# bacpop/Pansim

Hardware: AMD Instinct MI355X
Metric: generations/sec (higher is better)
Workload: dtype u8

## Files before the change

### pansim_amd/csrc/core_kernels.h

```cpp
#pragma once

#include "ps_common.h"

#include <type_traits>

#define PS_SWEEP_MAX_GENS 2
struct core_sweep_args {
    uint8_t *state;
    uint8_t *out;
    const uint32_t *idx;
    const uint32_t *idx_next[PS_SWEEP_MAX_GENS - 1];
    const uint32_t *idxT;
    uint32_t N, pitch, cpr, rows;
    uint32_t site_offset;
    uint32_t gen, k0, k1;
    ps_core_plan plan;
    uint32_t *overflow_flag;
    unsigned long long *stamps;
    uint32_t *work_ctr;
    uint32_t launch_parity;
    uint32_t nt;
    uint32_t qcap;
    uint32_t qcap_limit;
    uint32_t *wide_flags;
// ... 123 lines not shown
                    d[j] = w;
                }
            } else {
                const uint4 v = *(const uint4 *)(grow + 16u * c);
                d[0] = v.x; d[1] = v.y; d[2] = v.z; d[3] = v.w;
            }
            uint32_t hm = 0;
            if (events) {
                const ps_u4 A = ps_philox_l1a(site >> 1, c, a.gen, a.k0, a.k1), B = ps_philox_l1b(site >> 2, c, a.gen, a.k0, a.k1);
                uint32_t cm = ps_cand_word(A, site, pl.cshift);
                while (cm) {
                    const uint32_t k = ps_bit_cell(__builtin_ctz(cm));
                    cm &= cm - 1u;
                    const uint32_t i = c * 16u + k;
                    if (i >= a.N) continue;
                    uint32_t l2y;
                    const ps_cell cell = ps_cell_events<WT>(a, A, B, site, i, a.gen, a.k0, a.k1, pl, l2y);
                    if (DO_MUT && cell.mut) ps_set_byte(d, k, cell.mut);
                    if (DO_HR && cell.hr) hm |= 1u << k;
                }
            }
            if (DO_HR) {
                *(uint4 *)(rowS + 16u * c) = make_uint4(d[0], d[1], d[2], d[3]);
                hrm[c] = (uint16_t)hm;
            } else {
                *(uint4 *)(grow + 16u * c) = make_uint4(d[0], d[1], d[2], d[3]);
            }
        }
        if (DO_HR) {
            __syncthreads();
            for (uint32_t c = lane; c < a.cpr; c += lpr) {
                const uint4 v = *(const uint4 *)(rowS + 16u * c);
                uint32_t d[4] = { v.x, v.y, v.z, v.w };
                uint32_t hm = hrm[c];
                while (hm) {
                    const uint32_t k = __builtin_ctz(hm);
                    hm &= hm - 1u;
                    const uint32_t i = c * 16u + k;
                    const ps_u4 l2 = ps_philox(site, i, a.gen, PS_STREAM_CORE_L2, a.k0, a.k1);
                    uint32_t donor = ps_mulhi(l2.y, a.N - 1u);
                    donor += (donor >= i) ? 1u : 0u;
                    ps_set_byte(d, k, (uint32_t)rowS[donor]);
                }
                *(uint4 *)(grow + 16u * c) = make_uint4(d[0], d[1], d[2], d[3]);
            }
            if (!DO_GATHER) __syncthreads();
        }
    }
}

#define PS_BATCH_ROWS 4u

__device__ __forceinline__ void ps_wave_sync()
{
    __builtin_amdgcn_fence(__ATOMIC_RELEASE, "wavefront");
    __builtin_amdgcn_wave_barrier();
    __builtin_amdgcn_fence(__ATOMIC_ACQUIRE, "wavefront");
}

__device__ __forceinline__ uint32_t ps_lane_prefix(uint64_t bal)
{
    return __builtin_amdgcn_mbcnt_hi((uint32_t)(bal >> 32), __builtin_amdgcn_mbcnt_lo((uint32_t)bal, 0u));
}

__device__ __forceinline__ uint32_t ps_wave_scan_incl(uint32_t x)
{
    x += (uint32_t)__builtin_amdgcn_update_dpp(0, (int)x, 0x111, 0xF, 0xF, false);
    x += (uint32_t)__builtin_amdgcn_update_dpp(0, (int)x, 0x112, 0xF, 0xF, false);
    x += (uint32_t)__builtin_amdgcn_update_dpp(0, (int)x, 0x114, 0xF, 0xF, false);
    x += (uint32_t)__builtin_amdgcn_update_dpp(0, (int)x, 0x118, 0xF, 0xF, false);
    x += (uint32_t)__builtin_amdgcn_update_dpp(0, (int)x, 0x142, 0xA, 0xF, false);
    x += (uint32_t)__builtin_amdgcn_update_dpp(0, (int)x, 0x143, 0xC, 0xF, false);
    return x;
}

struct ps_class_words { uint32_t dec, res; };
__device__ __forceinline__ ps_class_words ps_classes(uint32_t p0, uint32_t p1, uint32_t p2, uint32_t p3, uint32_t p4, uint32_t p5,
                                                     uint32_t k, uint32_t nE, uint32_t vm)
{
    const uint32_t c1 = __builtin_amdgcn_bitop3_b32(p1, p2, p3, 0x01) & vm;
    uint32_t lt;
    switch (nE) {
    case 1: lt = __builtin_amdgcn_bitop3_b32(p0, p5, p4, 0x01); break;
    case 2: lt = __builtin_amdgcn_bitop3_b32(p0, p5, p4, 0x03); break;
    case 3: lt = __builtin_amdgcn_bitop3_b32(p0, p5, p4, 0x07); break;
    case 4: lt = __builtin_amdgcn_bitop3_b32(p0, p5, p4, 0x0F); break;
    case 5: lt = __builtin_amdgcn_bitop3_b32(p0, p5, p4, 0x1F); break;
    case 6: lt = __builtin_amdgcn_bitop3_b32(p0, p5, p4, 0x3F); break;
    case 7: lt = __builtin_amdgcn_bitop3_b32(p0, p5, p4, 0x7F); break;
    default: lt = 0xFFFFFFFFu; break;
    }
    ps_class_words o;
    o.dec = k ? c1 & __builtin_amdgcn_bitop3_b32(p0, p5, p4, 0x07) : 0u;
    o.res = c1 & lt & ~o.dec;
    return o;
}

struct ps_apply_words { uint32_t y0, y1, ya, yb, yc; };
PS_HD uint32_t ps_bfi(uint32_t m, uint32_t a, uint32_t b)
{
#if defined(__HIP_DEVICE_COMPILE__) && __has_builtin(__builtin_amdgcn_bitop3_b32)
    return __builtin_amdgcn_bitop3_b32(m, a, b, 0xCA);
#else
    return (a & m) | (b & ~m);
#endif
}
__device__ __forceinline__ ps_apply_words ps_apply_prepare(uint32_t dec, uint32_t p4, uint32_t p5)
{
    const uint32_t r1 = p5 >> 1, r2 = p4 >> 2, l1 = p5 << 1, l2 = dec << 2;
    ps_apply_words o;
    o.y0 = ps_bfi(0x01010101u, p4, ps_bfi(0x02020202u, l1, l2));
    o.y1 = ps_bfi(0x02020202u, p4, ps_bfi(0x04040404u, l1, l2));
    o.ya = ps_bfi(0x09090909u, r2, ps_bfi(0x12121212u, r1, dec));
    o.yb = ps_bfi(0x12121212u, r2, ps_bfi(0x24242424u, r1, dec));
    o.yc = ps_bfi(0x24242424u, r2, ps_bfi(0x48484848u, r1, dec));
    return o;
}
template <uint32_t SLOT>
__device__ __forceinline__ uint32_t ps_apply_dword(const ps_apply_words &y, uint32_t d)
{
    constexpr uint32_t sh = SLOT == 0u ? 0u : SLOT == 1u ? 1u : SLOT == 2u ? 0u : SLOT == 3u ? 1u : SLOT == 4u ? 2u : SLOT == 5u ? 3u : SLOT == 6u ? 4u : 5u;
    const uint32_t src = SLOT == 0u ? y.y0 : SLOT == 1u ? y.y1 : (SLOT == 2u || SLOT == 5u) ? y.ya : (SLOT == 3u || SLOT == 6u) ? y.yb : y.yc;
    const uint32_t f = (src >> sh) & 0x07070707u;
    const uint32_t allele = __builtin_amdgcn_perm(0x00080402u, 0u, f);
    const uint32_t mask = __builtin_amdgcn_perm(0x00FFFFFFu, 0u, f);
    return ps_bfi(mask, allele, d);
}
template <uint32_t H>
__device__ __forceinline__ void ps_apply_row(const ps_apply_words &y, uint4 &d)
{
    d.x = ps_apply_dword<4u * H + 0u>(y, d.x);
    d.y = ps_apply_dword<4u * H + 1u>(y, d.y);
    d.z = ps_apply_dword<4u * H + 2u>(y, d.z);
    d.w = ps_apply_dword<4u * H + 3u>(y, d.w);
}

__device__ __forceinline__ uint32_t ps_push_scan(uint32_t w0, uint32_t w1, uint16_t *q, uint32_t lane, uint32_t qcap)
{
    const uint32_t c0 = (uint32_t)__popc(w0), c = c0 + (uint32_t)__popc(w1);
    const uint32_t incl = ps_wave_scan_incl(c);
    const uint32_t qn = __builtin_amdgcn_readlane(incl, 63);
    if (qn <= qcap) {
        uint16_t *qp = q + (incl - c) - 1, *qp1 = qp + c0;
        const uint32_t tag = lane << 6;
        for (uint32_t m = w0; m; m &= m - 1u) *++qp = (uint16_t)(tag | (uint32_t)__builtin_ctz(m));
        for (uint32_t m = w1; m; m &= m - 1u) *++qp1 = (uint16_t)(tag | 32u | (uint32_t)__builtin_ctz(m));
    }
    return qn;
}
__device__ __forceinline__ uint32_t ps_entry_cell(uint32_t ent)
{
    const uint32_t cell = ((ent & 3u) << 2) | ((ent >> 3) & 3u), row = ((ent >> 2) & 1u) | ((ent >> 4) & 2u);
    return (row << 10) | ((ent >> 2) & 0x3F0u) | cell;
}

__device__ __forceinline__ uint32_t ps_pack4(uint32_t b0, uint32_t b1, uint32_t b2, uint32_t b3)
{
    return __builtin_amdgcn_perm(b1, b0, 0x0c0c0400u) | __builtin_amdgcn_perm(b3, b2, 0x04000c0cu);
}

#ifdef PS_STAMP
#define PS_T(k) do { unsigned long long t_; asm volatile("s_waitcnt lgkmcnt(0)\n\ts_memtime %0\n\ts_waitcnt lgkmcnt(0)" : "=s"(t_) :: "memory"); st_acc[k] += t_ - st_last; st_last = t_; } while (0)
#else
#define PS_T(k) do { } while (0)
#endif
#ifndef PS_WAVE_LB
#define PS_WAVE_LB 6
#endif
#ifndef PS_WAVE_PREFETCH
#define PS_WAVE_PREFETCH 0
#endif
__host__ __device__ constexpr uint32_t ps_queue_bytes(uint32_t qcap) { return (qcap * 2u + 15u) & ~15u; }
__host__ __device__ constexpr uint32_t ps_wave_lds(uint32_t qcap) { return PS_BATCH_ROWS * 1024u + ps_queue_bytes(qcap); }

template <bool DO_GATHER, bool DO_MUT, bool DO_HR, bool NT = false, bool WT = false, uint32_t T = 1>
__global__ void __launch_bounds__(256, T > 1 ? 4 : PS_WAVE_LB) core_sweep_wave_kernel(core_sweep_args a)
{
    static_assert(T >= 1 && T <= PS_SWEEP_MAX_GENS, "generations per pass");
    static_assert(T == 1 || (DO_GATHER && (DO_MUT || DO_HR)), "several generations per pass: the gather + events form only");
#ifdef PS_STAMP
    unsigned long long st_acc[8] = { 0, 0, 0, 0, 0, 0, 0, 0 };
    unsigned long long st_last;
    asm volatile("s_memtime %0\n\ts_waitcnt lgkmcnt(0)" : "=s"(st_last) :: "memory");
#endif
#ifdef PS_GROUP_TIMES
    const unsigned long long gt_start = __builtin_amdgcn_s_memrealtime();
#endif
    constexpr uint32_t PS_ROWS = PS_BATCH_ROWS;
    extern __shared__ __attribute__((aligned(16))) uint8_t lds[];
    const uint32_t wave = threadIdx.x >> 6, lane = threadIdx.x & 63u;
    uint8_t *rowbuf = lds + wave * ps_wave_lds(a.qcap);
    uint16_t *q = (uint16_t *)(rowbuf + PS_ROWS * 1024u);
    const ps_core_plan pl = a.plan;
    const uint32_t nE = 3u * pl.k + pl.R;
    constexpr bool events = DO_MUT || DO_HR;
    const bool has_chunk = lane < a.cpr;
    const uint32_t i0 = lane * 16u;
    const uint32_t ld_off = has_chunk ? i0 : 0u;
    const uint32_t nvalid = (i0 >= a.N) ? 0u : min(16u, a.N - i0);
    const uint32_t vm = ps_valid_word(nvalid);

    uint32_t pidx[T][16];
    if (DO_GATHER) {
#pragma unroll
        for (uint32_t t = 0; t < T; t++) {
            const uint32_t *ix = t ? a.idx_next[t ? t - 1u : 0u] : a.idx;
#pragma unroll
            for (uint32_t k = 0; k < 16; k++) pidx[t][k] = (k < nvalid) ? ix[i0 + k] : min(a.N, a.pitch - 1u);
        }
    }

    constexpr uint32_t PS_CHUNK = 3u;
    const uint32_t grp = blockIdx.x & 7u;
    const uint32_t off = a.site_offset & 3u, g0 = a.site_offset >> 2;
    const uint32_t batches = (a.rows + off + PS_ROWS - 1u) / PS_ROWS;
    const uint32_t b_lo = (uint32_t)((uint64_t)batches * grp / 8u), b_hi = (uint32_t)((uint64_t)batches * (grp + 1u) / 8u);
    uint32_t *ctr = a.work_ctr + (a.launch_parity * 8u + grp) * 32u;
    if (blockIdx.x < 8u && threadIdx.x == 0) a.work_ctr[((a.launch_parity ^ 1u) * 8u + blockIdx.x) * 32u] = 0u;
    uint32_t next_chunk = 0;
    if (lane == 0) next_chunk = __hip_atomic_fetch_add(ctr, 1u, __ATOMIC_RELAXED, __HIP_MEMORY_SCOPE_AGENT);
#if PS_WAVE_PREFETCH
    uint4 vn[PS_ROWS];
    uint32_t pf_batch = 0xFFFFFFFFu;
#pragma unroll
    for (uint32_t rr = 0; rr < PS_ROWS; rr++) vn[rr] = make_uint4(0, 0, 0, 0);
#endif
    for (;;) {
        const uint32_t chunk = __builtin_amdgcn_readfirstlane(next_chunk);
        if (b_lo + chunk * PS_CHUNK >= b_hi) break;
        if (lane == 0) next_chunk = __hip_atomic_fetch_add(ctr, 1u, __ATOMIC_RELAXED, __HIP_MEMORY_SCOPE_AGENT);
    for (uint32_t cb = 0; cb < PS_CHUNK; cb++) {
        const uint32_t batch = b_lo + chunk * PS_CHUNK + cb;
        if (batch >= b_hi) break;
        const int lr0 = (int)(batch * PS_ROWS) - (int)off;
        const uint32_t sg = g0 + batch;
        auto lrow = [&](uint32_t rr) -> uint32_t { return (uint32_t)min(max(lr0 + (int)rr, 0), (int)a.rows - 1); };
        uint4 v[PS_ROWS];
#if PS_WAVE_PREFETCH
        if (pf_batch == batch) {
#pragma unroll
            for (uint32_t rr = 0; rr < PS_ROWS; rr++) v[rr] = vn[rr];
        } else
#endif
#pragma unroll
        for (uint32_t rr = 0; rr < PS_ROWS; rr++)
            v[rr] = ps_load_row16(a.state + (size_t)lrow(rr) * a.pitch + ld_off, NT);
        if (DO_GATHER) {
#pragma unroll
            for (uint32_t rr = 0; rr < PS_ROWS; rr++) *(uint4 *)(rowbuf + rr * 1024u + i0) = v[rr];
            ps_wave_sync();
        }
        PS_T(0);

#pragma unroll
        for (uint32_t t = 0; t < T; t++) {
        const uint32_t gen = a.gen + t;
        uint32_t wl[2] = { 0u, 0u };
        ps_apply_words y[2] = {};
        if (events) {
            const ps_u4 A0 = ps_philox_l1a(2u * sg, lane, gen, a.k0, a.k1);
            const ps_u4 A1 = ps_philox_l1a(2u * sg + 1u, lane, gen, a.k0, a.k1);
            const ps_u4 B = ps_philox_l1b(sg, lane, gen, a.k0, a.k1);
            const ps_class_words c0 = ps_classes(A0.x, A0.y, A0.z, A0.w, B.x, B.z, pl.k, nE, vm);
            const ps_class_words c1 = ps_classes(A1.x, A1.y, A1.z, A1.w, B.y, B.w, pl.k, nE, vm);
            wl[0] = c0.res;
            wl[1] = c1.res;
            if (DO_MUT) {
                y[0] = ps_apply_prepare(c0.dec, B.x & c0.dec, B.z & c0.dec);
                y[1] = ps_apply_prepare(c1.dec, B.y & c1.dec, B.w & c1.dec);
            }
        }
        PS_T(2);
#pragma unroll
        for (uint32_t rr = 0; rr < PS_ROWS; rr++) {
            uint8_t *row = rowbuf + rr * 1024u;
            uint4 d = v[rr];
            if (DO_GATHER) {
                uint32_t w[4];
#pragma unroll
                for (int j = 0; j < 4; j++)
                    w[j] = ps_pack4(row[pidx[t][4 * j]], row[pidx[t][4 * j + 1]], row[pidx[t][4 * j + 2]], row[pidx[t][4 * j + 3]]);
                d = make_uint4(w[0], w[1], w[2], w[3]);
            }
            if (events && DO_MUT) {
                if (rr & 1u) ps_apply_row<1u>(y[rr >> 1], d);
                else ps_apply_row<0u>(y[rr >> 1], d);
            }
            if (DO_GATHER) ps_wave_sync();
            if (DO_GATHER || events) *(uint4 *)(row + i0) = d;
            __builtin_amdgcn_sched_barrier(0);
        }
        PS_T(1);
        const uint32_t qcap = a.qcap_limit ? min(a.qcap, a.qcap_limit) : a.qcap;
        uint32_t qn = 0;
        if (events) qn = ps_push_scan(wl[0], wl[1], q, lane, qcap);
        PS_T(3);
        ps_wave_sync();
#if PS_WAVE_PREFETCH
        if (t + 1u == T) {
            uint32_t nb = batch + 1u;
            if (cb + 1u >= PS_CHUNK || nb >= b_hi) nb = b_lo + (uint32_t)__builtin_amdgcn_readfirstlane(next_chunk) * PS_CHUNK;
            pf_batch = nb < b_hi ? nb : 0xFFFFFFFFu;
            if (nb < b_hi) {
                const int nlr0 = (int)(nb * PS_ROWS) - (int)off;
#pragma unroll
                for (uint32_t rr = 0; rr < PS_ROWS; rr++)
                    vn[rr] = ps_load_row16(a.state + (size_t)(uint32_t)min(max(nlr0 + (int)rr, 0), (int)a.rows - 1) * a.pitch + ld_off, NT);
            }
        }
#endif
        const bool redo = events && (qn > qcap || (DO_HR && 2u * qn > qcap));
        if (redo) {
#pragma unroll 1
            for (uint32_t rr = 0; rr < PS_ROWS; rr++) {
                uint8_t *row = rowbuf + rr * 1024u;
                const uint32_t site = 4u * sg + rr;
                const ps_u4 Ar = ps_philox_l1a(site >> 1, lane, gen, a.k0, a.k1);
                const ps_u4 Br = ps_philox_l1b(sg, lane, gen, a.k0, a.k1);
                uint32_t cmr = ps_cand_word(Ar, site, pl.cshift) & vm;
                uint32_t hm = 0;
                while (cmr) {
                    const uint32_t k = ps_bit_cell(__builtin_ctz(cmr)), cellidx = i0 + k;
                    cmr &= cmr - 1u;
                    uint32_t l2y = 0;
                    const ps_cell cell = ps_cell_events<WT>(a, Ar, Br, site, cellidx, gen, a.k0, a.k1, pl, l2y);
                    if (DO_MUT && cell.mut) row[cellidx] = (uint8_t)cell.mut;
                    if (DO_HR && cell.hr) hm |= 1u << k;
                }
                if (DO_HR) {
                    ps_wave_sync();
                    uint32_t dv[4] = { 0u, 0u, 0u, 0u };
                    for (uint32_t tmp = hm; tmp;) {
                        const uint32_t k = __builtin_ctz(tmp), cellidx = i0 + k;
                        tmp &= tmp - 1u;
                        const ps_u4 l2 = ps_philox(site, cellidx, gen, PS_STREAM_CORE_L2, a.k0, a.k1);
                        uint32_t donor = ps_mulhi(l2.y, a.N - 1u);
                        donor += (donor >= cellidx) ? 1u : 0u;
                        ps_set_byte(dv, k, (uint32_t)row[donor]);
                    }
                    ps_wave_sync();
                    for (uint32_t tmp = hm; tmp;) {
                        const uint32_t k = __builtin_ctz(tmp);
                        tmp &= tmp - 1u;
                        row[i0 + k] = (uint8_t)((dv[k >> 2] >> (8u * (k & 3u))) & 0xFFu);
                    }
                }
            }
            ps_wave_sync();
        } else if (events) {
            uint16_t *qh = q + qcap - 1u;
            for (uint32_t base = 0; base < qn; base += 64u) {
                const uint32_t e = base + lane;
                if (e < qn) {
                    const uint32_t ent = ps_entry_cell(q[e]);
                    const uint32_t cellidx = ent & 1023u, rr = ent >> 10;
                    const ps_u4 l2 = ps_philox(4u * sg + rr, cellidx, gen, PS_STREAM_CORE_L2, a.k0, a.k1);
                    const ps_cell cell = ps_classify_site<WT>(l2.x, pl, a, 4u * sg + rr);
                    if (DO_MUT && cell.mut) rowbuf[ent] = (uint8_t)cell.mut;
                    if (DO_HR) {
                        uint32_t out = 0;
                        if (cell.hr) {
                            uint32_t donor = ps_mulhi(l2.y, a.N - 1u);
                            donor += (donor >= cellidx) ? 1u : 0u;
                            out = donor | 0x8000u;
                        }
                        *(qh - e) = (uint16_t)out;
                    }
                }
            }
            if (DO_HR) {
                ps_wave_sync();
                for (uint32_t base = 0; base < qn; base += 64u) {
                    const uint32_t e = base + lane;
                    if (e < qn) {
                        const uint32_t h = *(qh - e);
                        if (h >> 15) *(qh - e) = (uint16_t)((uint32_t)rowbuf[(ps_entry_cell(q[e]) & 3072u) | (h & 1023u)] | 0x8000u);
                    }
                }
                ps_wave_sync();
                for (uint32_t base = 0; base < qn; base += 64u) {
                    const uint32_t e = base + lane;
                    if (e < qn) {
                        const uint32_t h = *(qh - e);
                        if (h >> 15) rowbuf[ps_entry_cell(q[e])] = (uint8_t)(h & 0xFFu);
                    }
                }
            }
            ps_wave_sync();
        }
        }
        PS_T(5);

        if (has_chunk) {
#pragma unroll
            for (uint32_t rr = 0; rr < PS_ROWS; rr++) {
                const int lr = lr0 + (int)rr;
                if (lr >= 0 && lr < (int)a.rows) {
                    const uint4 o = (DO_GATHER || events) ? *(const uint4 *)(rowbuf + rr * 1024u + i0) : v[rr];
                    ps_store_row16(a.out + (size_t)lr * a.pitch + i0, o, NT);
                }
            }
        }
        ps_wave_sync();
        PS_T(6);
    }
    }
#ifdef PS_STAMP
    if (lane == 0)
        for (int k = 0; k < 8; k++) atomicAdd((unsigned long long *)a.stamps + k, st_acc[k]);
#endif
#ifdef PS_GROUP_TIMES
    if (lane == 0) {
        atomicMax((unsigned long long *)a.stamps + 8 + grp, (unsigned long long)__builtin_amdgcn_s_memrealtime());
        atomicMax((unsigned long long *)a.stamps + 16 + grp, gt_start);
        if (blockIdx.x < 8 && wave == 0) ((unsigned long long *)a.stamps)[24 + grp] = gt_start;
    }
#endif
}

#ifndef PS_WCAP
#define PS_WCAP 1216u
#endif
#ifndef PS_WBPC
#define PS_WBPC 6
#endif
#ifndef PS_WLB
#define PS_WLB 6
#endif
#ifndef PS_WINDOW_NT_LOADS
#define PS_WINDOW_NT_LOADS 0
#endif
#define PS_WSTRIDE (PS_WCAP + 16u)
#define PS_WHR 64u
__host__ __device__ constexpr uint32_t ps_window_lds(uint32_t qcap) { return PS_BATCH_ROWS * PS_WSTRIDE + ps_queue_bytes(qcap) + PS_WHR * 6u; }

template <bool WT>
__device__ __forceinline__ uint32_t ps_donor_value(const core_sweep_args &a, const ps_core_plan &pl, const uint8_t *old_row,
                                                   uint32_t site, uint32_t donor, bool do_mut)
{
    uint32_t val = old_row[a.idx[donor]];
    if (do_mut) {
        const ps_u4 A = ps_philox_l1a(site >> 1, donor >> 4, a.gen, a.k0, a.k1);
// ... 1631 lines not shown
```

### pansim_amd/csrc/pansim_capi.hip

```cpp
#include "../../include/pansim_hip.h"

#include <hip/hip_runtime.h>

#include <algorithm>
#include <charconv>
#include <chrono>
#include <condition_variable>
#include <mutex>
#include <cmath>
#include <cstdarg>
#include <cstdio>
#include <cstdlib>
#include <cstring>
#include <string>
#include <thread>
#include <type_traits>
#include <vector>

#include "acc_kernels.h"
#include "core_kernels.h"
#include "ps_common.h"

static thread_local std::string g_err;

// ... 3054 lines not shown
    int32_t *h_num_genes = nullptr, *m_num_genes = nullptr;
    double *h_logw = nullptr, *m_logw = nullptr, *h_avg = nullptr;
    double *d_avg = nullptr;
    bool avg_prefetched = false;
    uint64_t avg_epoch = 0;
    hipEvent_t ev_avg = nullptr;
    std::vector<double> h_w;
    hipEvent_t ev_bin = nullptr;
    double *d_log1p = nullptr;
    uint64_t step_count = 0;
    uint64_t gens_done = 0;
    bool need_logw = false;
    bool device_draw = false;
    double *h_cum = nullptr, *d_cum = nullptr;
    uint32_t *d_idx_tsum = nullptr;
    uint32_t *d_idx_cnt = nullptr;
    int last_slot = 0;
    uint32_t *d_anc = nullptr;
    uint32_t anc_capacity = 0;
    uint64_t anc_written = 0;
    uint32_t *h_cnt = nullptr;
    uint64_t h_cnt_cap = 0;
    hipEvent_t ev_dist[4] = {};
    double dist_core_ms = 0.0, dist_acc_ms = 0.0;
    uint64_t host_calls = 0;
    double host_wait_ms = 0.0, host_weights_ms = 0.0, host_draw_ms = 0.0;
    int (*weights_hook)(void *ctx, ps_sim *s, uint32_t gen, double *w) = nullptr;
    void *weights_ctx = nullptr;
    int emu_shards = 0;
    void *emu_buf = nullptr;
    uint64_t emu_cap = 0;
    uint32_t emu_clock_khz = 0;
    double emu_link_gbps = 153.0, emu_latency_us = 20.0, emu_modelled_us = 0.0;
    uint64_t exchange_calls = 0, exchange_bytes = 0;
    bool timing = false;
    std::vector<std::pair<hipEvent_t, hipEvent_t>> tev;
    std::vector<hipEvent_t> ev_pool;
};

extern "C" void ps_sim_destroy(ps_sim *s)
{
    if (!s) return;
    if (s->core) (void)hipSetDevice(s->core->device);
    if (s->core) (void)hipStreamSynchronize(s->core->stream);
    if (s->acc) (void)hipStreamSynchronize(s->acc->stream);
    for (int k = 0; k < PS_RING; k++) {
        if (s->d_idx[k]) (void)hipFree(s->d_idx[k]);
        if (s->h_idx[k]) (void)hipHostFree(s->h_idx[k]);
        if (s->h_draw[k]) (void)hipHostFree(s->h_draw[k]);
        if (s->ev_idx[k]) (void)hipEventDestroy(s->ev_idx[k]);
        if (s->ev_core[k]) (void)hipEventDestroy(s->ev_core[k]);
        if (k == 0 && s->ev_hgt) (void)hipEventDestroy(s->ev_hgt);
        if (k == 0 && s->ev_avg) (void)hipEventDestroy(s->ev_avg);
        if (k == 0 && s->ev_bin) (void)hipEventDestroy(s->ev_bin);
        for (int j = 0; j < 2; j++) if (s->ev_gap[k][j]) (void)hipEventDestroy(s->ev_gap[k][j]);
    }
    if (s->h_num_genes) (void)hipHostFree(s->h_num_genes);
    if (s->h_logw) (void)hipHostFree(s->h_logw);
    if (s->h_avg) (void)hipHostFree(s->h_avg);
    if (s->h_cum) (void)hipHostFree(s->h_cum);
    if (s->d_cum) (void)hipFree(s->d_cum);
    if (s->d_idx_cnt) (void)hipFree(s->d_idx_cnt);
    if (s->d_idx_tsum) (void)hipFree(s->d_idx_tsum);
    if (s->d_anc) (void)hipFree(s->d_anc);
    if (s->h_cnt) (void)hipHostFree(s->h_cnt);
    for (auto e : s->ev_dist) if (e) (void)hipEventDestroy(e);
    if (s->d_avg) (void)hipFree(s->d_avg);
    if (s->emu_buf) (void)hipFree(s->emu_buf);
    if (s->d_log1p) (void)hipFree(s->d_log1p);
    for (auto &pr : s->tev) { (void)hipEventDestroy(pr.first); (void)hipEventDestroy(pr.second); }
    for (auto e : s->ev_pool) (void)hipEventDestroy(e);
    ps_population_destroy(s->core);
    ps_population_destroy(s->acc);
    delete s;
}

static int sim_refresh_rows(void *ctx);
static uint32_t sim_sweep_generations(ps_sim *s);

static int sim_create_impl(const ps_sim_params *p, ps_sim *s)
{
    char msg[1024];
    if (ps_sim_validate(p, msg, sizeof msg) != PS_OK) return ps_fail(PS_ERR_INVALID, "%s", msg);
    if (p->shard_count < 1 || p->shard_rank < 0 || p->shard_rank >= p->shard_count)
        return ps_fail(PS_ERR_INVALID, "bad shard %d of %d", p->shard_rank, p->shard_count);
    if (p->pop_size < 2) return ps_fail(PS_ERR_INVALID, "pop_size must be >= 2 (main.rs:421 / population.rs:584 panic)");
    s->prm = *p;
    PSCHK(ps_sim_derive(p, &s->der));
    const ps_derived &d = s->der;
    const uint64_t N = p->pop_size, L = p->core_size, G = d.pan_size;
    s->sel.assign(std::max<uint64_t>(G, 1), 0.0);
    if (p->reference_seed_stream)
        PSCHK(ps_reference_selection_coefficients(p->seed, G, p->prop_positive, p->pos_lambda, p->neg_lambda, s->sel.data()));
    else
        PSCHK(ps_selection_coefficients(p->seed, G, p->prop_positive, p->pos_lambda, p->neg_lambda, s->sel.data()));
    for (uint64_t g = 0; g < G; g++)
        if (std::log(1.0 + s->sel[g]) != 0.0) s->need_logw = true;
    const uint64_t sb = L * (uint64_t)p->shard_rank / (uint64_t)p->shard_count;
    const uint64_t se = L * ((uint64_t)p->shard_rank + 1) / (uint64_t)p->shard_count;
    ps_config cc{};
    cc.pop_size = N; cc.ncols = se - sb; cc.global_cols = L; cc.col_offset = sb;
    cc.core_genes = p->core_genes; cc.seed = p->seed; cc.core = 1; cc.device = p->device;
    {
        std::vector<uint8_t> v(std::max<uint64_t>(cc.ncols, 1));
        PSCHK(ps_init_vector(p->seed, 1, sb, cc.ncols, 0.0, v.data()));
        PSCHK(ps_population_create(&cc, v.data(), &s->core));
    }
    ps_config ca{};
    ca.pop_size = N; ca.ncols = G; ca.global_cols = G; ca.col_offset = 0;
    ca.core_genes = p->core_genes; ca.seed = p->seed; ca.core = 0; ca.device = s->core->device;
    {
        std::vector<uint8_t> v(std::max<uint64_t>(G, 1));
        PSCHK(ps_init_vector(p->seed, 0, 0, G, d.avg_gene_freq_adj, v.data()));
        PSCHK(ps_population_create(&ca, v.data(), &s->acc));
    }
    s->core->rows_refresh = s->acc->rows_refresh = sim_refresh_rows;
    s->core->rows_ctx = s->acc->rows_ctx = s;
    {
        const uint64_t b0 = 0, e0 = L;
        const double lm = d.n_core_mutations;
        const double lr = (p->HR_rate > 0.0) ? d.n_recombinations_core : 0.0;
        PSCHK(ps_set_rates(s->core, 1, &lm, &lr, &b0, &e0));
        double lrec[2] = { 0, 0 };
        for (int c = 0; c < d.n_comp; c++) lrec[c] = (p->HGT_rate > 0.0) ? d.n_recombinations_pan[c] : 0.0;
        PSCHK(ps_set_rates(s->acc, d.n_comp, d.n_pan_mutations, lrec, d.comp_begin, d.comp_end));
    }
    s->r1.resize(p->max_distances);
    s->r2.resize(p->max_distances);
    PSCHK(ps_sample_pairs(p->seed, N, p->max_distances, s->r1.data(), s->r2.data()));
    PSCHK(use_device(s->core));
    for (int k = 0; k < PS_RING; k++) {
        HIPCHK(hipMalloc(&s->d_idx[k], N * sizeof(uint32_t)));
        HIPCHK(hipHostMalloc(&s->h_idx[k], N * sizeof(uint32_t), hipHostMallocMapped));
        HIPCHK(hipHostGetDevicePointer((void **)&s->m_idx[k], s->h_idx[k], 0));
        HIPCHK(hipHostMalloc(&s->h_draw[k], N * sizeof(uint32_t), hipHostMallocMapped));
        HIPCHK(hipHostGetDevicePointer((void **)&s->m_draw[k], s->h_draw[k], 0));
        HIPCHK(hipEventCreateWithFlags(&s->ev_idx[k], hipEventDisableTiming));
        HIPCHK(hipEventCreateWithFlags(&s->ev_core[k], hipEventDisableTiming));
    }
    if (p->max_distances > 0) {
        PSCHK(upload_pairs(s->core, p->max_distances, s->r1.data(), s->r2.data(), true));
        PSCHK(upload_pairs(s->acc, p->max_distances, s->r1.data(), s->r2.data(), true));
    }
    if (!wave_sweep_eligible(s->core, true, p->HR_rate > 0.0)) {
        core_block_geom g{};
        uint32_t lds = 0, nw = 0;
        if (block_sweep_geometry(s->core, true, true, p->HR_rate > 0.0, &g, &lds, &nw))
            s->acc->hgt_list_in_global = lds + 16384u > s->core->lds_limit;
    }
    {
        const double bytes = 2.0 * (double)N * (double)s->core->cfg.ncols;
        double ept;
        if (sim_sweep_generations(s) >= 2u) {
            const double per_gen_ms = bytes / 3.7e12 * 1e3 / 2.0;
            ept = std::min((0.95 * per_gen_ms - 0.25) / 0.4e-3, 192.0);
        } else {
            const double sweep_ms = bytes / 4.2e12 * 1e3;
            ept = std::min((sweep_ms - 0.3) / 1.0e-3 * 0.5, 112.0);
        }
        s->acc->hgt_events_per_thread = ept >= 16.0 ? (uint32_t)ept : 0u;
        if (const char *e = getenv("PANSIM_HGT_EVENTS_PER_THREAD")) s->acc->hgt_events_per_thread = (uint32_t)atoi(e);
    }
    HIPCHK(hipEventCreateWithFlags(&s->ev_hgt, hipEventDisableTiming));
    {
        const uint32_t parts = hgt_partitions(s->acc);
        s->heavy_hgt = (double)N * s->der.n_recombinations_pan_total >= 7.5e6 && parts >= 1 && parts <= 1024;
    }
    if (const char *e = getenv("PANSIM_HEAVY_HGT")) s->heavy_hgt = atoi(e) != 0;
    if (!getenv("PANSIM_SWEEP_BLOCKS_PER_CU")) {
        uint64_t max_comp = 0;
        for (int c = 0; c < d.n_comp; c++) max_comp = std::max<uint64_t>(max_comp, d.comp_end[c] - d.comp_begin[c]);
        const uint64_t list_lds = 2 * max_comp;
        if (list_lds > 36 * 1024) s->acc->hgt_list_in_global = true;
        const uint32_t light = 4u;
        s->core->sweep_blocks_per_cu = list_lds <= 16 * 1024 ? light : std::min(light, 6u);
    }
    HIPCHK(hipHostMalloc(&s->h_num_genes, N * sizeof(int32_t), hipHostMallocMapped));
    HIPCHK(hipHostMalloc(&s->h_logw, N * sizeof(double), hipHostMallocMapped));
    HIPCHK(hipHostGetDevicePointer((void **)&s->m_num_genes, s->h_num_genes, 0));
    HIPCHK(hipHostGetDevicePointer((void **)&s->m_logw, s->h_logw, 0));
    HIPCHK(hipHostMalloc(&s->h_avg, N * sizeof(double)));
    s->device_draw = N >= 4096;
    if (const char *e = getenv("PANSIM_DEVICE_DRAW")) s->device_draw = atoi(e) != 0;
    HIPCHK(hipHostMalloc(&s->h_cum, N * sizeof(double)));
    HIPCHK(hipMalloc(&s->d_cum, N * sizeof(double)));
    HIPCHK(hipMalloc(&s->d_idx_tsum, ((N + 1023) / 1024 + 1) * sizeof(uint32_t)));
    HIPCHK(hipMalloc(&s->d_idx_cnt, N * sizeof(uint32_t)));
    HIPCHK(hipMemset(s->d_idx_cnt, 0, N * sizeof(uint32_t)));
    HIPCHK(hipMalloc(&s->d_avg, N * sizeof(double)));
    if (G) {
        std::vector<double> l1p(G);
        for (uint64_t g = 0; g < G; g++) l1p[g] = std::log(1.0 + s->sel[g] * 1.0);
        HIPCHK(hipMalloc(&s->d_log1p, G * sizeof(double)));
        HIPCHK(hipMemcpy(s->d_log1p, l1p.data(), G * sizeof(double), hipMemcpyHostToDevice));
    }
    if (G && !s->need_logw && !(getenv("PANSIM_FUSE_COUNTS") && atoi(getenv("PANSIM_FUSE_COUNTS")) == 0)) {
        s->acc->fuse_counts_out = s->m_num_genes;
        s->acc->fuse_logw_out = s->m_logw;
    }
    return PS_OK;
}

extern "C" int ps_sim_create(const ps_sim_params *p, ps_sim **out)
{
    if (!p || !out) return ps_fail(PS_ERR_INVALID, "null argument");
    *out = nullptr;
    ps_sim *s = new ps_sim();
    const int rc = sim_create_impl(p, s);
    if (rc != PS_OK) {
        const std::string keep = g_err;
        ps_sim_destroy(s);
        g_err = keep;
        return rc;
    }
    *out = s;
    return PS_OK;
}

static int sim_average_distance(ps_sim *s)
{
    ps_population *acc = s->acc;
    const uint64_t N = s->prm.pop_size;
    hipStream_t sa = acc->stream;
    const bool sharded = acc->exchange && acc->donor_cnt != 0 && acc->d.G > 0 && N >= 2;
    if (!sharded) return average_distance_device(acc, s->d_avg, sa);
    HIPCHK(hipMemsetAsync(s->d_avg, 0, N * sizeof(double), sa));
    PSCHK(average_distance_device(acc, s->d_avg, sa, acc->donor_lo, acc->donor_cnt));
    const std::string prev = g_err;
    g_err.clear();
    const int rc = acc->exchange(acc->exchange_ctx, s->d_avg, N, (void *)sa);
    if (rc != 0) {
        const std::string inner = g_err;
        return ps_fail(PS_ERR_STATE, "the all-gather of the average distances failed (%d)%s%s", rc, inner.empty() ? "" : ": ", inner.c_str());
    }
    g_err = prev;
    return PS_OK;
}

static int sim_host_weights(ps_sim *s, uint32_t gen, double *w, bool avg_ready = false)
{
    (void)gen;
    ps_population *acc = s->acc;
    const ps_sim_params &p = s->prm;
    const uint64_t N = p.pop_size;
    hipStream_t sa = acc->stream;
    using clk = std::chrono::steady_clock;
    auto ms_since = [](clk::time_point t0) { return std::chrono::duration<double, std::milli>(clk::now() - t0).count(); };
    for (uint64_t i = 0; i < N; i++) s->h_avg[i] = 1.0;
    if (p.competition_strength > 0.0) {
        const bool ahead = s->avg_prefetched && s->avg_epoch == acc->edit_epoch;
        if (!avg_ready && !ahead) PSCHK(sim_average_distance(s));
        s->avg_prefetched = false;
        HIPCHK(hipMemcpyAsync(s->h_avg, s->d_avg, N * sizeof(double), hipMemcpyDeviceToHost, sa));
    }
    if (s->need_logw)
        acc_fitness_kernel<<<(uint32_t)((N + 255) / 256), 256, 0, sa>>>(acc->I[acc->cur], s->d_log1p, 1,
                                                                     s->m_num_genes, s->m_logw, acc->d);
    else if (!acc->counts_fresh)
        acc_gene_count_rows_kernel<<<(uint32_t)((N + 3) / 4), 256, 0, sa>>>(acc->I[acc->cur], s->m_num_genes,
                                                                         s->m_logw, acc->d);
    HIPCHK(hipGetLastError());
    auto th0 = clk::now();
    HIPCHK(hipStreamSynchronize(sa));
    s->host_wait_ms += ms_since(th0);
    th0 = clk::now();
    PSCHK(ps_sample_weights(s->h_num_genes, s->h_logw, N, acc->cfg.ncols, s->der.avg_gene_num, s->h_avg,
                            p.no_control_genome_size, p.genome_size_penalty, p.competition_strength, w));
    s->host_weights_ms += ms_since(th0);
    return PS_OK;
}

static int sim_light_hgt(ps_sim *s, uint32_t gen)
{
    const bool heavy_hgt = s->prm.HGT_rate > 0.0 && s->heavy_hgt;
    if (s->prm.HGT_rate > 0.0 && !heavy_hgt) PSCHK(launch_acc_hgt(s->acc, gen, s->acc->stream));
    return PS_OK;
}

static int sim_accessory_half(ps_sim *s, uint32_t gen, uint32_t gens, bool light_hgt)
{
    ps_population *core = s->core, *acc = s->acc;
    const ps_sim_params &p = s->prm;
    const uint64_t N = p.pop_size, G = acc->cfg.ncols;
    hipStream_t sa = acc->stream, sc = core->stream;
    const int slot = (int)(s->step_count % PS_RING);
    using clk = std::chrono::steady_clock;
    auto ms_since = [](clk::time_point t0) { return std::chrono::duration<double, std::milli>(clk::now() - t0).count(); };
    auto th0 = clk::now();
    {
        const int back = (int)std::min<uint32_t>(4u * gens, PS_RING);
        const int wslot = (slot + PS_RING - back) % PS_RING;
        if (s->slot_used[wslot]) HIPCHK(hipEventSynchronize(s->ev_core[wslot]));
    }
    s->host_wait_ms += ms_since(th0);
    std::vector<double> &w = s->h_w;
    w.resize(N);
    if (s->weights_hook) PSCHK(s->weights_hook(s->weights_ctx, s, gen, w.data()));
    else PSCHK(sim_host_weights(s, gen, w.data()));
    th0 = clk::now();
    s->prev_slot = s->step_count ? s->last_slot : -1;
    s->last_slot = slot;
    if (core->rows_overridden || acc->rows_overridden) s->anc_written = 0;
    core->rows_overridden = acc->rows_overridden = false;
    const bool want_snap = p.HGT_rate > 0.0 && !hgt_takes_binned_form(acc);
    if (s->device_draw) {
        double total = w[0];
        for (uint64_t i = 1; i < N; i++) { s->h_cum[i - 1] = total; total += w[i]; }
        HIPCHK(hipMemcpyAsync(s->d_cum, s->h_cum, (N - 1) * sizeof(double), hipMemcpyHostToDevice, sa));
// ... 1042 lines not shown
```

Baseline: 3078.

## Interleave gather layout, vectorize index loads, and prefetch next row's LDS gather

Changes the per-lane child mapping in the gather so each lane handles four strided dwords (lane + 64*m) instead of a contiguous 16-byte chunk. This lets parent indices load as aligned uint4 vectors, and each packed dword is written back to LDS separately. For multi-generation sweeps, the LDS gather for the next row is issued ahead of time so its latency overlaps the current row's work. The HGT events-per-thread heuristic constants are also retuned. The cost is extra wave syncs and an LDS reload of the row when mutation is on, plus more registers held for the prefetched gather values.

```diff
diff --git a/pansim_amd/csrc/core_kernels.h b/pansim_amd/csrc/core_kernels.h
--- a/pansim_amd/csrc/core_kernels.h
+++ b/pansim_amd/csrc/core_kernels.h
@@ -299,6 +299,13 @@
 {
     const uint32_t cell = ((ent & 3u) << 2) | ((ent >> 3) & 3u), row = ((ent >> 2) & 1u) | ((ent >> 4) & 2u);
     return (row << 10) | ((ent >> 2) & 0x3F0u) | cell;
+}
+
+PS_HD uint32_t ps_gather_dword(uint32_t lane, uint32_t m) { return lane + 64u * m; }
+PS_HD uint32_t ps_gather_child(uint32_t lane, uint32_t m, uint32_t b) { return 4u * ps_gather_dword(lane, m) + b; }
+PS_HD uint32_t ps_gather_source(uint32_t child, uint32_t parent, uint32_t N, uint32_t pitch)
+{
+    return child < N ? parent : (N < pitch - 1u ? N : pitch - 1u);
 }
 
 __device__ __forceinline__ uint32_t ps_pack4(uint32_t b0, uint32_t b1, uint32_t b2, uint32_t b3)
@@ -352,8 +359,18 @@
 #pragma unroll
         for (uint32_t t = 0; t < T; t++) {
             const uint32_t *ix = t ? a.idx_next[t ? t - 1u : 0u] : a.idx;
-#pragma unroll
-            for (uint32_t k = 0; k < 16; k++) pidx[t][k] = (k < nvalid) ? ix[i0 + k] : min(a.N, a.pitch - 1u);
+            const bool wide = ((uintptr_t)ix & 15u) == 0u;
+#pragma unroll
+            for (uint32_t m = 0; m < 4; m++) {
+                const uint32_t c0 = ps_gather_child(lane, m, 0u);
+                if (wide && c0 + 4u <= a.N) {
+                    const uint4 p4 = *(const uint4 *)(ix + c0);
+                    pidx[t][4u * m] = p4.x, pidx[t][4u * m + 1u] = p4.y, pidx[t][4u * m + 2u] = p4.z, pidx[t][4u * m + 3u] = p4.w;
+                } else {
+#pragma unroll
+                    for (uint32_t b = 0; b < 4; b++) pidx[t][4u * m + b] = ps_gather_source(c0 + b, c0 + b < a.N ? ix[c0 + b] : 0u, a.N, a.pitch);
+                }
+            }
         }
     }
 
@@ -418,23 +435,40 @@
             }
         }
         PS_T(2);
+        constexpr bool ahead = T > 1 && DO_GATHER;
+        uint32_t g[16] = {};
+        auto gather = [&](uint32_t rr) {
+#pragma unroll
+            for (int k = 0; k < 16; k++) g[k] = rowbuf[rr * 1024u + pidx[t][k]];
+        };
+        if (ahead) gather(0u);
 #pragma unroll
         for (uint32_t rr = 0; rr < PS_ROWS; rr++) {
             uint8_t *row = rowbuf + rr * 1024u;
             uint4 d = v[rr];
             if (DO_GATHER) {
+                if (!ahead) gather(rr);
                 uint32_t w[4];
 #pragma unroll
-                for (int j = 0; j < 4; j++)
-                    w[j] = ps_pack4(row[pidx[t][4 * j]], row[pidx[t][4 * j + 1]], row[pidx[t][4 * j + 2]], row[pidx[t][4 * j + 3]]);
-                d = make_uint4(w[0], w[1], w[2], w[3]);
+                for (int m = 0; m < 4; m++) w[m] = ps_pack4(g[4 * m], g[4 * m + 1], g[4 * m + 2], g[4 * m + 3]);
+                ps_wave_sync();
+#pragma unroll
+                for (uint32_t m = 0; m < 4; m++) *(uint32_t *)(row + 4u * ps_gather_dword(lane, m)) = w[m];
+                if (events && DO_MUT) {
+                    ps_wave_sync();
+                    d = *(const uint4 *)(row + i0);
+                }
+                if (ahead && rr + 1u < PS_ROWS) {
+                    __builtin_amdgcn_sched_barrier(0);
+                    gather(rr + 1u);
+                    __builtin_amdgcn_sched_barrier(0);
+                }
             }
             if (events && DO_MUT) {
                 if (rr & 1u) ps_apply_row<1u>(y[rr >> 1], d);
                 else ps_apply_row<0u>(y[rr >> 1], d);
             }
-            if (DO_GATHER) ps_wave_sync();
-            if (DO_GATHER || events) *(uint4 *)(row + i0) = d;
+            if (events && (DO_MUT || !DO_GATHER)) *(uint4 *)(row + i0) = d;
             __builtin_amdgcn_sched_barrier(0);
         }
         PS_T(1);
diff --git a/pansim_amd/csrc/pansim_capi.hip b/pansim_amd/csrc/pansim_capi.hip
--- a/pansim_amd/csrc/pansim_capi.hip
+++ b/pansim_amd/csrc/pansim_capi.hip
@@ -3230,8 +3230,8 @@
         const double bytes = 2.0 * (double)N * (double)s->core->cfg.ncols;
         double ept;
         if (sim_sweep_generations(s) >= 2u) {
-            const double per_gen_ms = bytes / 3.7e12 * 1e3 / 2.0;
-            ept = std::min((0.95 * per_gen_ms - 0.25) / 0.4e-3, 192.0);
+            const double per_gen_ms = bytes / 4.0e12 * 1e3 / 2.0;
+            ept = std::min((per_gen_ms - 0.222) / 0.445e-3, 192.0);
         } else {
             const double sweep_ms = bytes / 4.2e12 * 1e3;
             ept = std::min((sweep_ms - 0.3) / 1.0e-3 * 0.5, 112.0);
```

After: 3252 (median of 6 runs). 5.7% higher.
